# BurntSushi/suffix

Hardware: AMD Instinct MI355X
Metric: MB of input text/sec for SuffixTable::new (SA-IS+LCP), 1 GPU; bit-exact SA (higher is better)
Workload: dtype u32; 1 GPU; 100000000 B synthetic DNA (sigma=4, uniform, splitmix64) per GPU, u32 indices, device-resident text -> device SA; text_bytes_total=100000000

## Files before the change

### suffix_amd/csrc/sfx_host.hpp

```cpp
#pragma once
#include <cstring>
#include <hip/hip_runtime.h>
#include <stdint.h>
#include <stdlib.h>

#include "../../include/suffix_hip.h"
#include "sfx_device.hpp"

namespace sfx {

void note_hip_error(hipError_t e, const char* what, const char* file, int line);

#define SFX_HIP(expr)                                                   \
    do {                                                                \
        hipError_t e_ = (expr);                                         \
        if (e_ != hipSuccess) {                                         \
            ::sfx::note_hip_error(e_, #expr, __FILE__, __LINE__);       \
            return SFX_ERR_HIP;                                         \
        }                                                               \
    } while (0)

#define SFX_TRY(expr)                       \
    do {                                    \
        int s_ = (expr);                    \
// ... 43 lines not shown
};
inline unsigned grid_cap()
{
    static const unsigned cap = [] {
        const char* e = dev_env("SFX_MAX_GRID");
        int v = e ? atoi(e) : 0;
        return (v >= 1 && v <= (int)kMaxGrid) ? (unsigned)v : kMaxGrid;
    }();
    return cap;
}
inline Chunking make_chunking(uint64_t items, uint64_t tile, unsigned max_blocks = kMaxGrid)
{
    Chunking c;
    if (max_blocks > grid_cap()) max_blocks = grid_cap();
    c.tiles = (items + tile - 1) / tile;
    if (c.tiles == 0) c.tiles = 1;
    c.tiles_per_block = (c.tiles + max_blocks - 1) / max_blocks;
    c.blocks = (unsigned)((c.tiles + c.tiles_per_block - 1) / c.tiles_per_block);
    return c;
}

bool profile_on();
void profile_begin(const char* name, hipStream_t st, double algo_bytes);
void profile_end(hipStream_t st);

#define SFX_LAUNCH(name, algo_bytes, kernel, grid, block, stream, ...)                  \
    do {                                                                                \
        if (::sfx::profile_on()) ::sfx::profile_begin(name, stream, (double)(algo_bytes)); \
        hipLaunchKernelGGL(kernel, dim3(grid), dim3(block), 0, stream, __VA_ARGS__);    \
        if (::sfx::profile_on()) ::sfx::profile_end(stream);                            \
        SFX_HIP(hipGetLastError());                                                     \
    } while (0)

#ifndef SFX_EMULATED
namespace detail {
constexpr unsigned kPostWords = 64;
static __global__ void __launch_bounds__(64) k_post_words(const uint32_t* __restrict__ src, unsigned words, volatile uint32_t* host,
                                                   uint32_t seq)
{
    const unsigned lane = threadIdx.x;
    if (lane < words) host[lane] = src[lane];
    __threadfence_system();
    __builtin_amdgcn_s_waitcnt(0);
    if (lane == 0) host[kPostWords] = seq;
}
}
#endif
inline int read_back(void* dst, const void* d_src, size_t bytes, hipStream_t st)
{
    constexpr size_t kStage = 4096, kPostArea = 512;
    thread_local void* stage = nullptr;
    thread_local bool tried = false;
    if (!tried) {
        tried = true;
        if (hipHostMalloc(&stage, kStage + kPostArea, hipHostMallocPortable | hipHostMallocMapped | hipHostMallocCoherent) != hipSuccess) {
            stage = nullptr;
            (void)hipGetLastError();
        }
        if (stage) std::memset(stage, 0, kStage + kPostArea);
    }
#ifndef SFX_EMULATED
    thread_local uint32_t seq = 0;
    if (stage && bytes > 0 && bytes <= detail::kPostWords * 4 && (bytes & 3u) == 0 && (reinterpret_cast<uintptr_t>(d_src) & 3u) == 0) {
        static_assert((detail::kPostWords + 16) * 4 <= kPostArea, "payload + the sequence word's own 64-byte block");
        volatile uint32_t* const host = reinterpret_cast<volatile uint32_t*>(static_cast<char*>(stage) + kStage);
        if (++seq == 0) seq = 1;
        hipLaunchKernelGGL(detail::k_post_words, dim3(1), dim3(64), 0, st, static_cast<const uint32_t*>(d_src), (unsigned)(bytes / 4), host, seq);
        SFX_HIP(hipGetLastError());
        for (unsigned spins = 1;; spins++) {
            if (host[detail::kPostWords] == seq) break;
#if defined(__x86_64__) || defined(__i386__)
            __builtin_ia32_pause();
#endif
            if ((spins & 0xFFFu) == 0) {
                const hipError_t q = hipStreamQuery(st);
                if (q == hipErrorNotReady) continue;
                SFX_HIP(q);
                if (host[detail::kPostWords] == seq) break;
                SFX_HIP(hipStreamSynchronize(st));
                goto by_copy;
            }
        }
        for (size_t i = 0; i < bytes / 4; i++) static_cast<uint32_t*>(dst)[i] = host[i];
        return SFX_OK;
    }
by_copy:
#endif
    void* via = (stage && bytes <= kStage) ? stage : dst;
    SFX_HIP(hipMemcpyAsync(via, d_src, bytes, hipMemcpyDeviceToHost, st));
    SFX_HIP(hipStreamSynchronize(st));
    if (via != dst) std::memcpy(dst, via, bytes);
    return SFX_OK;
}

struct BuildStats;

uint64_t radix_scratch_words(uint64_t m);
struct TieRecords {
    bool produced;
    const uint32_t* tmask;
    uint32_t* lmask;
    uint32_t* hmask;
    bool want_keys;
};
int radix_sort_e64(uint64_t* e0, uint64_t* e1, uint64_t m, int bit_lo, int bit_hi, uint32_t* scratch,
                   hipStream_t st, int* result_in_1, sfx_build_stats* stats, const PackedText* text,
                   uint32_t* split_v, uint32_t** split_k_out, unsigned hist_blocks = 0, int elem_bits = 0, TieRecords* ties = nullptr);
unsigned radix_e64_presort_hist(uint64_t m, int bit_lo, int bit_hi);
bool radix_e64_hybrid_expected(uint64_t m, int key_bits);
inline uint32_t* radix_partial(uint32_t* scratch) { return scratch; }
int radix_sort_kv64(uint64_t* k0, uint32_t* v0, uint64_t* k1, uint32_t* v1, uint64_t m, int bit_lo,
                    int bit_hi, uint32_t* scratch, hipStream_t st, int* result_in_1,
                    sfx_build_stats* stats, const PackedText* text, uint32_t* last_v = nullptr, uint64_t kv12_cap = 0);
int radix_sort_ht64(uint64_t* k0, uint32_t* v0, uint64_t* k1, uint32_t* v1, uint64_t m, uint32_t* scratch, hipStream_t st,
                    int* result_in_1, sfx_build_stats* stats, const PackedText& text, const uint32_t* ht, uint32_t* last_v = nullptr,
                    uint64_t kv12_cap = 0, int ctx_sigma = 0);
struct LcpEmit;
struct SegSort {
    void* segs;
    void* tiles;
    uint32_t* tilehist;
    uint32_t* segexcl;
    uint32_t* status;
    uint64_t status_words;
    uint32_t* counters;
// ... 165 lines not shown
```

### suffix_amd/csrc/sfx_radix.hip

```cpp
#include <stdio.h>
#include <type_traits>
#include <stdlib.h>

#include "sfx_host.hpp"

namespace sfx {

constexpr uint32_t kStatusAgg = 1u << 30;
constexpr uint32_t kStatusPrefix = 2u << 30;
constexpr uint32_t kStatusValue = (1u << 30) - 1u;
constexpr int kMaxPasses = 8;
constexpr unsigned kHistAllGrid = 1024;

struct SrcE64 {
    static constexpr bool kHasVal = false;
    static constexpr bool kFromText = false;
    const uint64_t* in;
    __device__ __forceinline__ uint64_t key(uint64_t i) const { return in[i]; }
    __device__ __forceinline__ uint32_t val(uint64_t) const { return 0u; }
};
struct SrcText32 {
    static constexpr bool kHasVal = false;
    static constexpr bool kFromText = true;
    PackedText t;
    __device__ __forceinline__ uint64_t key(uint64_t i) const
    {
        return ((uint64_t)packed_key32(t, i) << 32) | (uint64_t)(uint32_t)i;
    }
    __device__ __forceinline__ uint32_t val(uint64_t) const { return 0u; }
};
struct SrcText36 {
    static constexpr bool kHasVal = false;
    static constexpr bool kFromText = true;
    PackedText t;
    int extra;
    bool wide;
    __device__ __forceinline__ uint64_t key(uint64_t i) const
    {
        uint64_t k64;
        if (wide) {
            k64 = packed_key64(t, i);
        } else {
            const uint64_t q = packed_word_index(t, i);
            const unsigned off = packed_word_offset(t, i, q);
            uint64_t pair;
            __builtin_memcpy(&pair, t.words + q, 8);
            const uint64_t both = ((pair & 0xFFFFFFFFull) << 32) | (pair >> 32);
            k64 = both << (off * (unsigned)t.bits);
        }
        return ((k64 >> (32 - extra)) << (32 - extra)) | (uint64_t)(uint32_t)i;
    }
    __device__ __forceinline__ uint32_t val(uint64_t) const { return 0u; }
};
struct SrcKV {
    static constexpr bool kHasVal = true;
    static constexpr bool kFromText = false;
    const uint64_t* k;
    const uint32_t* v;
    __device__ __forceinline__ uint64_t key(uint64_t i) const { return k[i]; }
    __device__ __forceinline__ uint32_t val(uint64_t i) const { return v[i]; }
};
struct SrcKeyIota {
    static constexpr bool kHasVal = true;
    static constexpr bool kFromText = false;
    const uint64_t* k;
    __device__ __forceinline__ uint64_t key(uint64_t i) const { return k[i]; }
    __device__ __forceinline__ uint32_t val(uint64_t i) const { return (uint32_t)i; }
};
struct SrcText64 {
    static constexpr bool kHasVal = true;
    static constexpr bool kFromText = true;
    PackedText t;
    __device__ __forceinline__ uint64_t key(uint64_t i) const { return packed_key64(t, i); }
    __device__ __forceinline__ uint32_t val(uint64_t i) const { return (uint32_t)i; }
};
struct DstE64 {
    uint64_t* out;
    __device__ __forceinline__ void store(uint32_t d, uint64_t key, uint32_t) const { out[d] = key; }
};
struct DstSplit32 {
    uint32_t* k;
    uint32_t* v;
    __device__ __forceinline__ void store(uint32_t d, uint64_t key, uint32_t) const
    {
        k[d] = (uint32_t)(key >> 32);
// ... 680 lines not shown
#pragma unroll
                for (int j = 0; j < kOut; j++) {
                    ok[j] = s.stage[(j0 + j) * kThreads + t];
                    ov[j] = HAS_VAL ? s.stage_v[(j0 + j) * kThreads + t] : 0u;
                }
#pragma unroll
                for (int j = 0; j < kOut; j++) od[j] = s.off[digit_of(ok[j], shift, mask)] + (unsigned)(h * kHalf + (j0 + j) * kThreads) + t;
#pragma unroll
                for (int j = 0; j < kOut; j++)
                    if ((unsigned)(h * kHalf + (j0 + j) * kThreads) + t < nvalid) dst.store(od[j], ok[j], ov[j]);
            }
        }
        if (owner) {
            unsigned col = tid;
            SFX_OPAQUE_VGPR(col);
#pragma unroll
            for (int k = 0; k < NW; k++) s.cnt[k][col] = 0;
        }
        __syncthreads();
    }
}

constexpr unsigned kCursorPad = 16;
constexpr unsigned kPartClasses = 8;
template <int KPT, int NW>
struct PartSmem {
    uint64_t stage[NW * kWave * KPT];
    uint16_t cnt[NW][kRadix];
    uint32_t off[kRadix];
    uint32_t tiles_before[kRadix];
    uint32_t class_tiles[8];
    uint32_t part[2][NW];
};
template <class Src, int KPT, int NW, bool SUB>
__global__ void __launch_bounds__(NW * kWave) SFX_WAVES_PER_EU(4, 4)
k_partition(Src src, uint64_t* __restrict__ out, uint64_t m, int shift, uint32_t* __restrict__ cursor,
            const uint32_t* __restrict__ bstart16, uint64_t class_len)
{
    constexpr int kThreads = NW * kWave;
    constexpr uint32_t kTile = kThreads * KPT;
    static_assert(kThreads >= kRadix, "thread d owns bucket d");
    static_assert(kWave * KPT >= kRadix, "the match masks must fit the staging buffer");
    static_assert(kTile < 65536, "16-bit tile positions");
    __shared__ PartSmem<KPT, NW> s;
    const unsigned tid = threadIdx.x, lane = lane_id(), w = wave_id();
    const unsigned long long mybit = 1ull << lane;
    const bool owner = tid < (unsigned)kRadix;
    unsigned par = 0;
    unsigned long long* const my_flags = reinterpret_cast<unsigned long long*>(s.stage) + w * kRadix;
    uint64_t ntiles;
    {
        const uint64_t first = dmin<uint64_t>(m, class_len);
        ntiles = ((first + kTile - 1) / kTile) * kPartClasses;
    }
    if (SUB) {
        if (owner) s.tiles_before[tid] = (bstart16[(tid + 1u) << 8] - bstart16[tid << 8] + kTile - 1u) / kTile;
        __syncthreads();
        if (tid < 8u) {
            uint32_t run = 0;
            for (unsigned b = tid; b < (unsigned)kRadix; b += 8u) {
                const uint32_t tb = s.tiles_before[b];
                s.tiles_before[b] = run;
                run += tb;
            }
            s.class_tiles[tid] = run;
        }
        __syncthreads();
        uint32_t most = 0;
#pragma unroll
        for (int x = 0; x < 8; x++) most = dmax(most, s.class_tiles[x]);
        ntiles = (uint64_t)most * 8u;
    }
    if (owner) {
#pragma unroll
        for (int k = 0; k < NW; k++) s.cnt[k][tid] = 0;
    }
    __syncthreads();
    auto locate = [&](uint64_t v, uint64_t& begin, unsigned& nvalid, unsigned& top) {
        begin = v * kTile;
        nvalid = 0;
        top = 0;
        if (v >= ntiles) return;
        if (SUB) {
            const unsigned x = (unsigned)(v & 7u);
            const uint32_t u = (uint32_t)(v >> 3);
            if (u >= s.class_tiles[x]) return;
            unsigned lo = 0, hi = kRadix / 8;
            while (hi - lo > 1u) {
                const unsigned mid = (lo + hi) / 2u;
                if (s.tiles_before[x + 8u * mid] <= u) lo = mid; else hi = mid;
            }
            top = x + 8u * lo;
            const uint32_t b0 = bstart16[top << 8], b1 = bstart16[(top + 1u) << 8];
            begin = (uint64_t)b0 + (uint64_t)(u - s.tiles_before[top]) * kTile;
            nvalid = (unsigned)dmin<uint64_t>(kTile, (uint64_t)b1 - begin);
        } else {
            const unsigned x = (unsigned)(v % kPartClasses);
            const uint64_t p0 = dmin<uint64_t>(m, (uint64_t)x * class_len), p1 = dmin<uint64_t>(m, p0 + class_len);
            begin = p0 + (v / kPartClasses) * kTile;
            top = x;
            if (begin < p1) nvalid = (unsigned)dmin<uint64_t>(kTile, p1 - begin);
        }
    };
    for (uint64_t v = blockIdx.x; v < ntiles; v += gridDim.x) {
        uint64_t begin;
        unsigned nvalid, top;
        locate(v, begin, nvalid, top);
        if (nvalid == 0u) continue;
        uint64_t key[KPT];
        uint32_t pos[KPT];
        unsigned first = w * (kWave * KPT) + lane;
        SFX_OPAQUE_VGPR(first);
#pragma unroll
        for (int r = 0; r < KPT; r++) {
            const unsigned idx = first + r * kWave;
            key[r] = idx < nvalid ? src.key(begin + idx) : ~0ull;
        }
#pragma unroll
        for (int k = 0; k < kRadix / kWave; k++) my_flags[k * kWave + lane] = 0ull;
        wave_sync();
#pragma unroll
        for (int r = 0; r < KPT; r++) pos[r] = rank_round16(digit_of(key[r], shift, 255u), my_flags, s.cnt[w], mybit);
        __syncthreads();
        uint32_t real_count = 0, tile_ex = 0, mine = 0;
        {
            uint32_t c[NW], tile_count = 0;
#pragma unroll
            for (int k = 0; k < NW; k++) {
                c[k] = owner ? s.cnt[k][tid] : 0u;
                tile_count += c[k];
            }
            const uint32_t ex = block_scan_excl_1b<NW>(tile_count, s.part, par);
            if (owner) {
                uint32_t run = ex;
#pragma unroll
                for (int k = 0; k < NW; k++) {
                    s.cnt[k][tid] = (uint16_t)run;
                    run += c[k];
                }
                real_count = tile_count - ((tid == 255u) ? (uint32_t)(kTile - nvalid) : 0u);
                tile_ex = ex;
                if (real_count) mine = atomicAdd(&cursor[SUB ? ((top << 8) | tid) : (top * kRadix + tid) * kCursorPad], real_count);
            }
        }
        __syncthreads();
#pragma unroll
        for (int r = 0; r < KPT; r++) s.stage[pos[r] + s.cnt[w][digit_of(key[r], shift, 255u)]] = key[r];
        if (owner) s.off[tid] = mine - tile_ex;
        __syncthreads();
        constexpr int kOut = (KPT % 4 == 0) ? 4 : ((KPT % 2 == 0) ? 2 : 1);
        unsigned t = tid;
        SFX_OPAQUE_VGPR(t);
#pragma unroll
        for (int r0 = 0; r0 < KPT; r0 += kOut) {
#pragma unroll
            for (int r = r0; r < r0 + kOut; r++) key[r] = s.stage[r * kThreads + t];
#pragma unroll
            for (int r = r0; r < r0 + kOut; r++) pos[r] = s.off[digit_of(key[r], shift, 255u)] + ((unsigned)r * kThreads + t);
#pragma unroll
            for (int r = r0; r < r0 + kOut; r++)
                if ((unsigned)r * kThreads + t < nvalid) out[pos[r]] = key[r];
        }
        if (owner) {
#pragma unroll
            for (int k = 0; k < NW; k++) s.cnt[k][tid] = 0;
        }
        __syncthreads();
    }
}
__global__ void __launch_bounds__(kBlock)
k_partition_cursors(const uint32_t* __restrict__ bstart16, const uint32_t* __restrict__ class_top8, uint32_t* __restrict__ cursor16,
                    uint32_t* __restrict__ cursor8)
{
    const unsigned i = blockIdx.x * kBlock + threadIdx.x;
    if (i < (unsigned)(1 << 16)) {
        const uint32_t b = bstart16[i];
        cursor16[i] = b;
        if ((i & 255u) == 0u) {
            uint32_t run = b;
            for (unsigned x = 0; x < kPartClasses; x++) {
                cursor8[(x * kRadix + (i >> 8)) * kCursorPad] = run;
                run += class_top8[x * kRadix + (i >> 8)];
            }
        }
    }
}

constexpr int kH16Bins = 1 << 16;
constexpr int kH16Words = kH16Bins / 2;
constexpr int kH16Threads = 1024;
__global__ void __launch_bounds__(kH16Threads)
k_hist16_text(PackedText t, int drop, uint64_t words_per_block, uint32_t* __restrict__ partial)
{
    __shared__ uint32_t h[kH16Words];
    const unsigned tid = threadIdx.x;
    const uint64_t nwords = (t.n + (uint64_t)t.spw - 1) / (uint64_t)t.spw;
    const uint64_t qb = (uint64_t)blockIdx.x * words_per_block;
    const uint64_t qe = dmin<uint64_t>(nwords, qb + words_per_block);
    const uint64_t mask = (1ull << t.kbits) - 1ull;
    for (unsigned i = tid; i < (unsigned)kH16Words; i += kH16Threads) h[i] = 0;
    __syncthreads();
    for (uint64_t q = qb + tid; q < qe; q += kH16Threads) {
        const uint64_t both = ((uint64_t)t.words[q] << t.kbits) | (uint64_t)t.words[q + 1];
        const uint64_t j0 = q * (uint64_t)t.spw;
        for (int o = 0; o < t.spw; o++) {
            if (j0 + (uint64_t)o >= t.n) break;
            const uint32_t key = (uint32_t)((both >> ((unsigned)(t.spw - o) * (unsigned)t.bits)) & mask);
            const uint32_t top = key >> drop;
            atomicAdd(&h[top >> 1], (top & 1u) ? 65536u : 1u);
        }
    }
    __syncthreads();
    uint32_t* out = partial + (uint64_t)blockIdx.x * kH16Words;
    for (unsigned i = tid; i < (unsigned)kH16Words; i += kH16Threads) out[i] = h[i];
}
__global__ void __launch_bounds__(kH16Threads)
k_hist16_e64(const uint64_t* __restrict__ E, uint64_t m, int shift, uint64_t per_block, uint32_t* __restrict__ partial)
{
    __shared__ uint32_t h[kH16Words];
    const unsigned tid = threadIdx.x;
    const uint64_t qb = (uint64_t)blockIdx.x * per_block;
    const uint64_t qe = dmin<uint64_t>(m, qb + per_block);
    for (unsigned i = tid; i < (unsigned)kH16Words; i += kH16Threads) h[i] = 0;
    __syncthreads();
    constexpr int kFly = 8;
    for (uint64_t q0 = qb; q0 < qe; q0 += (uint64_t)kH16Threads * kFly) {
        uint64_t e[kFly];
#pragma unroll
        for (int k = 0; k < kFly; k++) {
            const uint64_t q = q0 + (uint64_t)k * kH16Threads + tid;
            e[k] = q < qe ? E[q] : ~0ull;
        }
#pragma unroll
        for (int k = 0; k < kFly; k++) {
            if (q0 + (uint64_t)k * kH16Threads + tid < qe) {
                const uint32_t top = (uint32_t)(e[k] >> shift) & 0xFFFFu;
                atomicAdd(&h[top >> 1], (top & 1u) ? 65536u : 1u);
            }
        }
    }
    __syncthreads();
    uint32_t* out = partial + (uint64_t)blockIdx.x * kH16Words;
    for (unsigned i = tid; i < (unsigned)kH16Words; i += kH16Threads) out[i] = h[i];
}
constexpr int kH16ReduceBins = 1024;
constexpr unsigned kH16ReduceSplit = 8;
__global__ void __launch_bounds__(kBlock)
k_hist16_reduce(const uint32_t* __restrict__ partial, unsigned nblocks, uint32_t* __restrict__ bins, unsigned rows_per_class,
                uint32_t* __restrict__ class_top8)
{
    const unsigned bx = blockIdx.x % (kH16Bins / kH16ReduceBins), by = blockIdx.x / (kH16Bins / kH16ReduceBins);
    const unsigned w0 = bx * (kH16ReduceBins / 2) + threadIdx.x * 2;
    uint32_t c[4] = {0, 0, 0, 0};
    const unsigned g1 = dmin(nblocks, (by + 1u) * rows_per_class);
    for (unsigned g = by * rows_per_class; g < g1; g++) {
        const uint2 v = *reinterpret_cast<const uint2*>(partial + (uint64_t)g * kH16Words + w0);
        c[0] += v.x & 0xFFFFu;
        c[1] += v.x >> 16;
        c[2] += v.y & 0xFFFFu;
        c[3] += v.y >> 16;
    }
#pragma unroll
    for (int k = 0; k < 4; k++)
        if (c[k]) atomicAdd(&bins[2 * w0 + k], c[k]);
    uint32_t all = c[0] + c[1] + c[2] + c[3];
    for (int d = 32; d >= 1; d >>= 1) all += __shfl_xor(all, d);
    static_assert(kWave * 4 == kRadix, "a wave's bins are one top-8 bucket");
    if (lane_id() == 0) class_top8[by * kRadix + (2u * w0) / (unsigned)kRadix] = all;
}
struct OversizeEntry { uint32_t bin, start, size, off; };
constexpr uint32_t kOversizeMax = 16384;
__global__ void __launch_bounds__(kH16Threads)
k_hist16_scan(uint32_t* __restrict__ bins, uint32_t* __restrict__ totals_lo, uint32_t* __restrict__ totals_hi,
              uint32_t* __restrict__ stat_out, uint32_t cap, uint32_t fast)
{
    __shared__ uint32_t part[kH16Threads / kWave];
    __shared__ uint32_t pmax[kH16Threads / kWave];
    __shared__ uint32_t lo[4][kRadix];
    __shared__ uint32_t tsum[kH16Threads];
    constexpr int kPer = kH16Bins / kH16Threads;
    const unsigned tid = threadIdx.x;
    {
        const unsigned d = tid & 255u, q = tid >> 8;
        uint32_t t = 0;
        for (unsigned j = q; j < (unsigned)kRadix; j += 4) t += bins[j * kRadix + d];
        lo[q][d] = t;
    }
    uint32_t v[kPer], sum = 0, most = 0;
    {
        uint32_t slow = 0, nover = 0, sover = 0;
        for (int j = 0; j < kPer; j++) {
            v[j] = bins[tid * kPer + j];
            sum += v[j];
            most = dmax(most, v[j]);
            if (v[j] > fast) slow += v[j];
            if (v[j] > cap) { nover++; sover += v[j]; }
        }
        if (slow) atomicAdd(&stat_out[4], slow);
        if (nover) { atomicAdd(&stat_out[2], nover); atomicAdd(&stat_out[3], sover); }
    }
    tsum[tid] = sum;
    for (int d = 32; d >= 1; d >>= 1) most = dmax(most, __shfl_xor(most, d));
    const uint32_t incl = wave_scan_add(sum);
    if (lane_id() == 63) part[wave_id()] = incl;
    if (lane_id() == 0) pmax[wave_id()] = most;
    __syncthreads();
    if (tid < (unsigned)kRadix) {
        totals_lo[tid] = lo[0][tid] + lo[1][tid] + lo[2][tid] + lo[3][tid];
        totals_hi[tid] = tsum[4 * tid] + tsum[4 * tid + 1] + tsum[4 * tid + 2] + tsum[4 * tid + 3];
    }
    uint32_t base = 0;
    for (unsigned k = 0; k < wave_id(); k++) base += part[k];
    uint32_t run = base + incl - sum;
    for (int j = 0; j < kPer; j++) { bins[tid * kPer + j] = run; run += v[j]; }
    if (tid == kH16Threads - 1) { bins[kH16Bins] = run; stat_out[1] = run; }
    if (tid == 0) {
        uint32_t mx = 0;
        for (unsigned k = 0; k < (unsigned)(kH16Threads / kWave); k++) mx = dmax(mx, pmax[k]);
        stat_out[0] = mx;
    }
}
__global__ void __launch_bounds__(kH16Threads)
k_hist16_oversize(const uint32_t* __restrict__ bstart, uint32_t cap, OversizeEntry* __restrict__ over)
{
    __shared__ uint64_t pover[kH16Threads / kWave];
    constexpr int kPer = kH16Bins / kH16Threads;
    const unsigned tid = threadIdx.x;
    uint64_t ov = 0;
    for (int j = 0; j < kPer; j++) {
        const uint32_t b = tid * kPer + j, v = bstart[b + 1] - bstart[b];
        if (v > cap) ov += (1ull << 32) | (uint64_t)v;
    }
    const uint64_t incl = wave_scan_add(ov);
    if (lane_id() == 63) pover[wave_id()] = incl;
    __syncthreads();
    uint64_t run = incl - ov;
    for (unsigned k = 0; k < wave_id(); k++) run += pover[k];
    if (ov == 0) return;
    for (int j = 0; j < kPer; j++) {
        const uint32_t b = tid * kPer + j, start = bstart[b], v = bstart[b + 1] - start;
        if (v > cap) {
            const uint32_t at = (uint32_t)(run >> 32);
            if (at < kOversizeMax) over[at] = OversizeEntry{b, start, v, (uint32_t)run};
            run += (1ull << 32) | (uint64_t)v;
        }
    }
}
__global__ void __launch_bounds__(kBlock)
k_oversize_gather(const uint64_t* __restrict__ X, const OversizeEntry* __restrict__ over, uint32_t nover, int low_bits,
                  uint64_t* __restrict__ T)
{
    const uint32_t lmask = (uint32_t)((1ull << low_bits) - 1ull);
// ... 374 lines not shown
bool radix_e64_hybrid_expected(uint64_t m, int key_bits)
{
    return hybrid_size_ok(m) && key_bits >= 24;
}
static int hybrid_sort_e64_text(uint64_t* e0, uint64_t* e1, uint64_t m, int bit_lo, int bit_hi, const RadixScratch& scr,
                                hipStream_t st, sfx_build_stats* stats, const PackedText& text, uint32_t* split_v,
                                uint32_t** split_k_out, bool* done, bool* windows_ready, int elem_bits = 0, TieRecords* ties = nullptr)
{
    if (ties) ties->produced = false;
    *done = false;
    *windows_ready = false;
    const bool from_elems = elem_bits > 0;
    static const uint32_t cap = [] {
        const char* e = dev_env("SFX_HYBRID_CAP");
        const uint32_t full = kBucketNW * kWave * kBucketKPT;
        const uint32_t v = e ? (uint32_t)atoi(e) : full;
        return v >= 1 && v < full ? v : full;
    }();
    const int key_bits = from_elems ? elem_bits : bit_hi - bit_lo;
    if (!hybrid_size_ok(m) || bit_lo != 32 || key_bits < 24 || key_bits > bit_hi - bit_lo) return SFX_OK;
    if (!from_elems && (key_bits != text.kbits || m != text.n)) return SFX_OK;
    const int low_bits = key_bits - 16;
    const int top_hi = bit_lo + key_bits;
    constexpr uint64_t kReserve = 1u << 18;
    uint32_t* bins = scr.partial + ((uint64_t)kMaxPasses * kRadix * kHistAllGrid - kReserve);
    uint32_t* stat = bins + kH16Bins + 64;
    OversizeEntry* over = reinterpret_cast<OversizeEntry*>(bins + kH16Bins + 128);
    static_assert(kH16Bins + 128 + 4 * kOversizeMax <= kReserve, "the reserve holds bins, statistics and the oversize list");
    uint32_t* partial = reinterpret_cast<uint32_t*>(e1);
    const uint64_t nwords = from_elems ? m : (m + (uint64_t)text.spw - 1) / (uint64_t)text.spw;
    const uint64_t room = m * sizeof(uint64_t) / (kH16Words * sizeof(uint32_t));
    if (room == 0) return SFX_OK;
    Chunking ch = make_chunking(nwords, kH16Threads, (unsigned)dmin<uint64_t>(room, 256));
    SFX_HIP(hipMemsetAsync(scr.tickets, 0, 64 * sizeof(uint32_t), st));
    SFX_HIP(hipMemsetAsync(bins, 0, (kH16Bins + 128) * sizeof(uint32_t), st));
    if (from_elems)
        SFX_LAUNCH("radix_hist16_elems", (double)m * 8.0, k_hist16_e64, ch.blocks, kH16Threads, st, (const uint64_t*)e0, m, top_hi - 16,
                   ch.tiles_per_block * kH16Threads, partial);
    else
        SFX_LAUNCH("radix_hist16_text", (double)m * text.bits / 8.0, k_hist16_text, ch.blocks, kH16Threads, st, text, low_bits,
                   ch.tiles_per_block * kH16Threads, partial);
    static_assert(kH16ReduceSplit == kPartClasses, "one block group of the reduction per stretch");
    const unsigned rows_per_class = (ch.blocks + kPartClasses - 1) / kPartClasses;
    const uint64_t class_len = (uint64_t)rows_per_class * ch.tiles_per_block * kH16Threads * (from_elems ? 1u : (uint64_t)text.spw);
    uint32_t* cursor16 = bins + kH16Bins + 128 + 4 * kOversizeMax;
    uint32_t* class_top8 = cursor16 + kH16Bins;
    uint32_t* cursor8 = class_top8 + kPartClasses * kRadix;
    static_assert(kH16Bins + 128 + 4 * kOversizeMax + kH16Bins + kPartClasses * kRadix * (1 + kCursorPad) <= kReserve, "the reserve holds the cursors too");
    SFX_LAUNCH("radix_hist16_reduce", (double)ch.blocks * kH16Words * 4, k_hist16_reduce, (kH16Bins / kH16ReduceBins) * kH16ReduceSplit, kBlock, st,
               (const uint32_t*)partial, ch.blocks, bins, rows_per_class, class_top8);
    SFX_LAUNCH("radix_hist16_scan", (double)kH16Bins * 8, k_hist16_scan, 1, kH16Threads, st, bins, scr.totals, scr.totals + kRadix,
               stat, cap, dmin(cap, 4096u));
    uint32_t host_stat[5] = {0, 0, 0, 0, 0};
    SFX_TRY(read_back(host_stat, stat, sizeof(host_stat), st));
    const uint32_t host_max = host_stat[0], nover = host_stat[2];
    const uint64_t nlarge = host_stat[3], nslow = host_stat[4];
    const bool give_way = nover > kOversizeMax || nslow * 64 > m ||
                          (nover && (m + 1) / 2 + 32 + 2 * (nlarge + 32) > m);
    if ((uint64_t)host_stat[1] != m) return SFX_OK;
    if (give_way) {
        if (!from_elems && text.kbits == 32 && (8 % text.bits) == 0 && bit_hi == 64) {
            SFX_HIP(hipMemsetAsync(scr.tickets, 0, 64 * sizeof(uint32_t), st));
            SFX_LAUNCH("radix_window_from_hist16", 0.0, k_window_from_hist16, 1, kBlock, st, scr.totals, (uint32_t)(3 * (8 / text.bits)));
            SFX_LAUNCH("radix_window_fix", 0.0, k_window_fix, 1, kBlock, st, text, scr.totals);
            *windows_ready = true;
        }
        return SFX_OK;
    }
    static const int ties_on = [] { const char* e = dev_env("SFX_HYBRID_TIES"); return e ? atoi(e) : 1; }();
    const bool tie_mode = ties && ties_on && nover == 0;
    static const int partition = [] { const char* e = dev_env("SFX_HYBRID_PARTITION"); return e ? atoi(e) : 1; }();
    static const int key36_on = [] { const char* e = dev_env("SFX_HYBRID_KEY36"); return e ? atoi(e) : 1; }();
    int extra = 0;
    if (tie_mode && key36_on && partition && !from_elems && text.kbits == 32 && text.bits <= 4 && m <= (1ull << 28))
        extra = key36_on >= 2 ? (4 / text.bits) * text.bits : text.bits;
    const bool wide_key = extra > text.bits;
    const int sbits = 32 - extra;
    if (partition) {
        constexpr int kPKpt = 16;
        SFX_LAUNCH("partition_cursors", (double)kH16Bins * 8, k_partition_cursors, kH16Bins / kBlock, kBlock, st, (const uint32_t*)bins,
                   (const uint32_t*)class_top8, cursor16, cursor8);
        static const unsigned cus = [] {
            int dev = 0, n = 0;
            if (hipGetDevice(&dev) != hipSuccess || hipDeviceGetAttribute(&n, hipDeviceAttributeMultiprocessorCount, dev) != hipSuccess || n <= 0) n = 256;
            return (unsigned)n;
        }();
        static const int pwaves = [] { const char* e = dev_env("SFX_PARTITION_WAVES"); const int v = e ? atoi(e) : 8; return (v == 16 || v == 4) ? v : 8; }();
        auto partition_pair = [&](auto nw) -> int {
            constexpr int kPNw = decltype(nw)::value;
            const uint64_t tile = (uint64_t)kPKpt * kPNw * kWave;
            const unsigned per_cu = 16u / kPNw;
            const unsigned g1 = (unsigned)dmin<uint64_t>((m + tile - 1) / tile, dmin(per_cu * cus, grid_cap()));
            const unsigned g2 = (unsigned)dmin<uint64_t>((m + tile - 1) / tile + kRadix, dmin(per_cu * cus, grid_cap()));
            if (from_elems) {
                SFX_LAUNCH("radix_scatter_u32", (double)m * 16.0, (k_partition<SrcE64, kPKpt, kPNw, false>), g1, kPNw * kWave, st,
                           SrcE64{e0}, e1, m, top_hi - 8, cursor8, (const uint32_t*)bins, class_len);
                SFX_LAUNCH("radix_scatter_u32", (double)m * 16.0, (k_partition<SrcE64, kPKpt, kPNw, true>), g2, kPNw * kWave, st,
                           SrcE64{e1}, e0, m, top_hi - 16, cursor16, (const uint32_t*)bins, class_len);
                uint64_t* t = e0; e0 = e1; e1 = t;
            } else {
                if (extra)
                    SFX_LAUNCH("radix_scatter_text_u32", (double)m * (text.bits / 8.0 + 8.0), (k_partition<SrcText36, kPKpt, kPNw, false>),
                               g1, kPNw * kWave, st, SrcText36{text, extra, wide_key}, e0, m, top_hi - 8, cursor8, (const uint32_t*)bins, class_len);
                else
                    SFX_LAUNCH("radix_scatter_text_u32", (double)m * (text.bits / 8.0 + 8.0), (k_partition<SrcText32, kPKpt, kPNw, false>),
                               g1, kPNw * kWave, st, SrcText32{text}, e0, m, top_hi - 8, cursor8, (const uint32_t*)bins, class_len);
                SFX_LAUNCH("radix_scatter_u32", (double)m * 16.0, (k_partition<SrcE64, kPKpt, kPNw, true>), g2, kPNw * kWave, st,
                           SrcE64{e0}, e1, m, top_hi - 16, cursor16, (const uint32_t*)bins, class_len);
            }
            return SFX_OK;
        };
        if (pwaves == 16) SFX_TRY(partition_pair(std::integral_constant<int, 16>{}));
        else if (pwaves == 4) SFX_TRY(partition_pair(std::integral_constant<int, 4>{}));
        else SFX_TRY(partition_pair(std::integral_constant<int, 8>{}));
    } else if (from_elems) {
        SFX_TRY(run_pass("radix_scatter_u32", (double)m * 16.0, SrcE64{e0}, DstE64{e1}, m, top_hi - 16, 255u, scr, 0, true, st));
        SFX_TRY(run_pass("radix_scatter_u32", (double)m * 16.0, SrcE64{e1}, DstE64{e0}, m, top_hi - 8, 255u, scr, 1, true, st));
        uint64_t* t = e0; e0 = e1; e1 = t;
    } else {
        SrcText32 tsrc = {text};
        SFX_TRY(run_pass("radix_scatter_text_u32", (double)m * (text.bits / 8.0 + 8.0), tsrc, DstE64{e0}, m, top_hi - 16, 255u, scr, 0,
                         true, st));
        SFX_TRY(run_pass("radix_scatter_u32", (double)m * 16.0, SrcE64{e0}, DstE64{e1}, m, top_hi - 8, 255u, scr, 1, true, st));
    }
    uint32_t* split_k = reinterpret_cast<uint32_t*>(e0);
    const uint64_t* over_sorted = nullptr;
    if (nover) {
        SFX_LAUNCH("radix_hist16_oversize", (double)kH16Bins * 8, k_hist16_oversize, 1, kH16Threads, st, (const uint32_t*)bins, cap, over);
        uint64_t* T = e0 + (((m + 1) / 2 + 31) & ~uint64_t(31));
        uint64_t* T2 = T + ((nlarge + 31) & ~uint64_t(31));
        const unsigned g = (unsigned)dmin<uint64_t>(nover, kMaxGrid);
        SFX_LAUNCH("oversize_gather", (double)nlarge * 16, k_oversize_gather, g, kBlock, st, (const uint64_t*)e1, (const OversizeEntry*)over,
                   nover, low_bits, T);
        int in1 = 0;
        SFX_TRY(radix_sort_e64(T, T2, nlarge, 32, 32 + low_bits + bits_for(nover > 1 ? nover - 1 : 1), scr.partial, st, &in1, stats,
                               nullptr, nullptr, nullptr, 0));
        over_sorted = in1 ? T2 : T;
    }
    static const int force_geom = [] { const char* e = dev_env("SFX_HYBRID_GEOM"); return e ? atoi(e) : -1; }();
// ... 681 lines not shown
```

Baseline: 76350 MB/s.

## Fuse radix hist16 reduce, scan and cursor setup; prefetch text words in partition

```diff
diff --git a/suffix_amd/csrc/sfx_host.hpp b/suffix_amd/csrc/sfx_host.hpp
--- a/suffix_amd/csrc/sfx_host.hpp
+++ b/suffix_amd/csrc/sfx_host.hpp
@@ -99,9 +99,11 @@
         SFX_HIP(hipGetLastError());                                                     \
     } while (0)
 
+namespace detail {
+constexpr unsigned kPostWords = 64;
+}
 #ifndef SFX_EMULATED
 namespace detail {
-constexpr unsigned kPostWords = 64;
 static __global__ void __launch_bounds__(64) k_post_words(const uint32_t* __restrict__ src, unsigned words, volatile uint32_t* host,
                                                    uint32_t seq)
 {
@@ -113,9 +115,14 @@
 }
 }
 #endif
-inline int read_back(void* dst, const void* d_src, size_t bytes, hipStream_t st)
-{
-    constexpr size_t kStage = 4096, kPostArea = 512;
+struct PostTicket {
+    volatile uint32_t* host;
+    uint32_t seq;
+};
+namespace detail {
+constexpr size_t kStage = 4096, kPostArea = 512;
+inline void* post_stage()
+{
     thread_local void* stage = nullptr;
     thread_local bool tried = false;
     if (!tried) {
@@ -126,14 +133,48 @@
         }
         if (stage) std::memset(stage, 0, kStage + kPostArea);
     }
+    return stage;
+}
+}
+inline PostTicket post_ticket()
+{
 #ifndef SFX_EMULATED
     thread_local uint32_t seq = 0;
-    if (stage && bytes > 0 && bytes <= detail::kPostWords * 4 && (bytes & 3u) == 0 && (reinterpret_cast<uintptr_t>(d_src) & 3u) == 0) {
-        static_assert((detail::kPostWords + 16) * 4 <= kPostArea, "payload + the sequence word's own 64-byte block");
-        volatile uint32_t* const host = reinterpret_cast<volatile uint32_t*>(static_cast<char*>(stage) + kStage);
+    void* const stage = detail::post_stage();
+    if (stage) {
+        static_assert((detail::kPostWords + 16) * 4 <= detail::kPostArea, "payload + the sequence word's own 64-byte block");
         if (++seq == 0) seq = 1;
-        hipLaunchKernelGGL(detail::k_post_words, dim3(1), dim3(64), 0, st, static_cast<const uint32_t*>(d_src), (unsigned)(bytes / 4), host, seq);
-        SFX_HIP(hipGetLastError());
+        return PostTicket{reinterpret_cast<volatile uint32_t*>(static_cast<char*>(stage) + detail::kStage), seq};
+    }
+#endif
+    return PostTicket{nullptr, 0};
+}
+template <class Words>
+__device__ __forceinline__ void post_words_from_kernel(const PostTicket& t, const Words& src, unsigned words)
+{
+#ifndef SFX_EMULATED
+    if (!t.host) return;
+    for (unsigned i = 0; i < words; i++) t.host[i] = src[i];
+    __threadfence_system();
+    __builtin_amdgcn_s_waitcnt(0);
+    t.host[detail::kPostWords] = t.seq;
+#endif
+}
+inline int read_by_copy(void* dst, const void* d_src, size_t bytes, hipStream_t st)
+{
+    void* const stage = detail::post_stage();
+    void* via = (stage && bytes <= detail::kStage) ? stage : dst;
+    SFX_HIP(hipMemcpyAsync(via, d_src, bytes, hipMemcpyDeviceToHost, st));
+    SFX_HIP(hipStreamSynchronize(st));
+    if (via != dst) std::memcpy(dst, via, bytes);
+    return SFX_OK;
+}
+inline int read_posted(void* dst, const void* d_src, size_t bytes, const PostTicket& t, hipStream_t st)
+{
+#ifndef SFX_EMULATED
+    if (t.host && bytes > 0 && bytes <= detail::kPostWords * 4 && (bytes & 3u) == 0) {
+        volatile uint32_t* const host = t.host;
+        const uint32_t seq = t.seq;
         for (unsigned spins = 1;; spins++) {
             if (host[detail::kPostWords] == seq) break;
 #if defined(__x86_64__) || defined(__i386__)
@@ -145,19 +186,29 @@
                 SFX_HIP(q);
                 if (host[detail::kPostWords] == seq) break;
                 SFX_HIP(hipStreamSynchronize(st));
-                goto by_copy;
+                return read_by_copy(dst, d_src, bytes, st);
             }
         }
         for (size_t i = 0; i < bytes / 4; i++) static_cast<uint32_t*>(dst)[i] = host[i];
         return SFX_OK;
     }
-by_copy:
-#endif
-    void* via = (stage && bytes <= kStage) ? stage : dst;
-    SFX_HIP(hipMemcpyAsync(via, d_src, bytes, hipMemcpyDeviceToHost, st));
-    SFX_HIP(hipStreamSynchronize(st));
-    if (via != dst) std::memcpy(dst, via, bytes);
-    return SFX_OK;
+#endif
+    return read_by_copy(dst, d_src, bytes, st);
+}
+inline int read_back(void* dst, const void* d_src, size_t bytes, hipStream_t st)
+{
+#ifndef SFX_EMULATED
+    if (bytes > 0 && bytes <= detail::kPostWords * 4 && (bytes & 3u) == 0 && (reinterpret_cast<uintptr_t>(d_src) & 3u) == 0) {
+        const PostTicket t = post_ticket();
+        if (t.host) {
+            hipLaunchKernelGGL(detail::k_post_words, dim3(1), dim3(64), 0, st, static_cast<const uint32_t*>(d_src), (unsigned)(bytes / 4), t.host,
+                               t.seq);
+            SFX_HIP(hipGetLastError());
+            return read_posted(dst, d_src, bytes, t, st);
+        }
+    }
+#endif
+    return read_by_copy(dst, d_src, bytes, st);
 }
 
 struct BuildStats;
diff --git a/suffix_amd/csrc/sfx_radix.hip b/suffix_amd/csrc/sfx_radix.hip
--- a/suffix_amd/csrc/sfx_radix.hip
+++ b/suffix_amd/csrc/sfx_radix.hip
@@ -28,6 +28,10 @@
         return ((uint64_t)packed_key32(t, i) << 32) | (uint64_t)(uint32_t)i;
     }
     __device__ __forceinline__ uint32_t val(uint64_t) const { return 0u; }
+    __device__ __forceinline__ uint64_t from_window(uint64_t k64, uint64_t i) const
+    {
+        return (k64 & 0xFFFFFFFF00000000ull) | (uint64_t)(uint32_t)i;
+    }
 };
 struct SrcText36 {
     static constexpr bool kHasVal = false;
@@ -48,9 +52,37 @@
             const uint64_t both = ((pair & 0xFFFFFFFFull) << 32) | (pair >> 32);
             k64 = both << (off * (unsigned)t.bits);
         }
+        return from_window(k64, i);
+    }
+    __device__ __forceinline__ uint32_t val(uint64_t) const { return 0u; }
+    __device__ __forceinline__ uint64_t from_window(uint64_t k64, uint64_t i) const
+    {
         return ((k64 >> (32 - extra)) << (32 - extra)) | (uint64_t)(uint32_t)i;
     }
-    __device__ __forceinline__ uint32_t val(uint64_t) const { return 0u; }
+};
+template <int SPW, int KPT>
+struct TextTileWords {
+    static_assert(SPW >= KPT ? SPW % KPT == 0 : KPT % SPW == 0, "a thread's positions begin on a word boundary or stay inside one word");
+    static constexpr int kOwn = SPW >= KPT ? 1 : KPT / SPW;
+    static constexpr int kCount = kOwn + 1;
+    uint32_t w[kCount];
+    __device__ __forceinline__ void load(const PackedText& t, uint64_t begin, unsigned tid)
+    {
+        __builtin_memcpy(w, t.words + (begin / (unsigned)SPW + ((uint64_t)tid * KPT) / (unsigned)SPW), sizeof(w));
+    }
+    template <class Src>
+    __device__ __forceinline__ void keys(const Src& src, uint64_t begin, unsigned tid, uint64_t (&key)[KPT]) const
+    {
+        constexpr unsigned kBits = 32u / SPW;
+        const unsigned off0 = SPW > KPT ? (tid * KPT) % (unsigned)SPW : 0u;
+#pragma unroll
+        for (int r = 0; r < KPT; r++) {
+            const int j = SPW > KPT ? 0 : r / SPW;
+            const unsigned off = SPW > KPT ? off0 + (unsigned)r : (unsigned)(r % SPW);
+            const uint64_t both = ((uint64_t)w[j] << 32) | (uint64_t)w[j + 1];
+            key[r] = src.from_window(both << (off * kBits), begin + (uint64_t)tid * KPT + (unsigned)r);
+        }
+    }
 };
 struct SrcKV {
     static constexpr bool kHasVal = true;
@@ -797,13 +829,14 @@
     uint32_t class_tiles[8];
     uint32_t part[2][NW];
 };
-template <class Src, int KPT, int NW, bool SUB>
+template <class Src, int KPT, int NW, bool SUB, int SPW = 0>
 __global__ void __launch_bounds__(NW * kWave) SFX_WAVES_PER_EU(4, 4)
 k_partition(Src src, uint64_t* __restrict__ out, uint64_t m, int shift, uint32_t* __restrict__ cursor,
             const uint32_t* __restrict__ bstart16, uint64_t class_len)
 {
     constexpr int kThreads = NW * kWave;
     constexpr uint32_t kTile = kThreads * KPT;
+    static_assert(SPW == 0 || (Src::kFromText && !SUB), "the tile loader reads packed text");
     static_assert(kThreads >= kRadix, "thread d owns bucket d");
     static_assert(kWave * KPT >= kRadix, "the match masks must fit the staging buffer");
     static_assert(kTile < 65536, "16-bit tile positions");
@@ -867,19 +900,42 @@
             if (begin < p1) nvalid = (unsigned)dmin<uint64_t>(kTile, p1 - begin);
         }
     };
+    TextTileWords<SPW ? SPW : KPT, KPT> words = {};
+    auto request = [&](uint64_t v) {
+        if constexpr (SPW > 0) {
+            uint64_t begin;
+            unsigned nvalid, top;
+            locate(v, begin, nvalid, top);
+            if (nvalid == kTile) words.load(src.t, begin, tid);
+        }
+    };
+    request(blockIdx.x);
     for (uint64_t v = blockIdx.x; v < ntiles; v += gridDim.x) {
         uint64_t begin;
         unsigned nvalid, top;
         locate(v, begin, nvalid, top);
-        if (nvalid == 0u) continue;
+        if (nvalid == 0u) {
+            request(v + gridDim.x);
+            continue;
+        }
         uint64_t key[KPT];
         uint32_t pos[KPT];
-        unsigned first = w * (kWave * KPT) + lane;
-        SFX_OPAQUE_VGPR(first);
-#pragma unroll
-        for (int r = 0; r < KPT; r++) {
-            const unsigned idx = first + r * kWave;
-            key[r] = idx < nvalid ? src.key(begin + idx) : ~0ull;
+        bool striped = true;
+        if constexpr (SPW > 0) {
+            if (nvalid == kTile) {
+                words.keys(src, begin, tid, key);
+                striped = false;
+            }
+            request(v + gridDim.x);
+        }
+        if (striped) {
+            unsigned first = w * (kWave * KPT) + lane;
+            SFX_OPAQUE_VGPR(first);
+#pragma unroll
+            for (int r = 0; r < KPT; r++) {
+                const unsigned idx = first + r * kWave;
+                key[r] = idx < nvalid ? src.key(begin + idx) : ~0ull;
+            }
         }
 #pragma unroll
         for (int k = 0; k < kRadix / kWave; k++) my_flags[k * kWave + lane] = 0ull;
@@ -933,30 +989,24 @@
         __syncthreads();
     }
 }
-__global__ void __launch_bounds__(kBlock)
-k_partition_cursors(const uint32_t* __restrict__ bstart16, const uint32_t* __restrict__ class_top8, uint32_t* __restrict__ cursor16,
-                    uint32_t* __restrict__ cursor8)
-{
-    const unsigned i = blockIdx.x * kBlock + threadIdx.x;
-    if (i < (unsigned)(1 << 16)) {
-        const uint32_t b = bstart16[i];
-        cursor16[i] = b;
-        if ((i & 255u) == 0u) {
-            uint32_t run = b;
-            for (unsigned x = 0; x < kPartClasses; x++) {
-                cursor8[(x * kRadix + (i >> 8)) * kCursorPad] = run;
-                run += class_top8[x * kRadix + (i >> 8)];
-            }
-        }
-    }
-}
-
 constexpr int kH16Bins = 1 << 16;
 constexpr int kH16Words = kH16Bins / 2;
 constexpr int kH16Threads = 1024;
+struct H16Zero {
+    uint32_t* a;
+    uint32_t na;
+    uint32_t* b;
+    uint32_t nb;
+    __device__ __forceinline__ void clear(unsigned threads) const
+    {
+        for (uint32_t i = blockIdx.x * threads + threadIdx.x; i < na; i += gridDim.x * threads) a[i] = 0;
+        for (uint32_t i = blockIdx.x * threads + threadIdx.x; i < nb; i += gridDim.x * threads) b[i] = 0;
+    }
+};
 __global__ void __launch_bounds__(kH16Threads)
-k_hist16_text(PackedText t, int drop, uint64_t words_per_block, uint32_t* __restrict__ partial)
-{
+k_hist16_text(PackedText t, int drop, uint64_t words_per_block, uint32_t* __restrict__ partial, H16Zero z)
+{
+    z.clear(kH16Threads);
     __shared__ uint32_t h[kH16Words];
     const unsigned tid = threadIdx.x;
     const uint64_t nwords = (t.n + (uint64_t)t.spw - 1) / (uint64_t)t.spw;
@@ -965,8 +1015,11 @@
     const uint64_t mask = (1ull << t.kbits) - 1ull;
     for (unsigned i = tid; i < (unsigned)kH16Words; i += kH16Threads) h[i] = 0;
     __syncthreads();
+    uint32_t w0 = 0, w1 = 0;
+    if (qb + tid < qe) { w0 = t.words[qb + tid]; w1 = t.words[qb + tid + 1]; }
     for (uint64_t q = qb + tid; q < qe; q += kH16Threads) {
-        const uint64_t both = ((uint64_t)t.words[q] << t.kbits) | (uint64_t)t.words[q + 1];
+        const uint64_t both = ((uint64_t)w0 << t.kbits) | (uint64_t)w1;
+        if (q + kH16Threads < qe) { w0 = t.words[q + kH16Threads]; w1 = t.words[q + kH16Threads + 1]; }
         const uint64_t j0 = q * (uint64_t)t.spw;
         for (int o = 0; o < t.spw; o++) {
             if (j0 + (uint64_t)o >= t.n) break;
@@ -980,8 +1033,9 @@
     for (unsigned i = tid; i < (unsigned)kH16Words; i += kH16Threads) out[i] = h[i];
 }
 __global__ void __launch_bounds__(kH16Threads)
-k_hist16_e64(const uint64_t* __restrict__ E, uint64_t m, int shift, uint64_t per_block, uint32_t* __restrict__ partial)
-{
+k_hist16_e64(const uint64_t* __restrict__ E, uint64_t m, int shift, uint64_t per_block, uint32_t* __restrict__ partial, H16Zero z)
+{
+    z.clear(kH16Threads);
     __shared__ uint32_t h[kH16Words];
     const unsigned tid = threadIdx.x;
     const uint64_t qb = (uint64_t)blockIdx.x * per_block;
@@ -1008,81 +1062,132 @@
     uint32_t* out = partial + (uint64_t)blockIdx.x * kH16Words;
     for (unsigned i = tid; i < (unsigned)kH16Words; i += kH16Threads) out[i] = h[i];
 }
-constexpr int kH16ReduceBins = 1024;
-constexpr unsigned kH16ReduceSplit = 8;
-__global__ void __launch_bounds__(kBlock)
-k_hist16_reduce(const uint32_t* __restrict__ partial, unsigned nblocks, uint32_t* __restrict__ bins, unsigned rows_per_class,
-                uint32_t* __restrict__ class_top8)
-{
-    const unsigned bx = blockIdx.x % (kH16Bins / kH16ReduceBins), by = blockIdx.x / (kH16Bins / kH16ReduceBins);
-    const unsigned w0 = bx * (kH16ReduceBins / 2) + threadIdx.x * 2;
-    uint32_t c[4] = {0, 0, 0, 0};
-    const unsigned g1 = dmin(nblocks, (by + 1u) * rows_per_class);
-    for (unsigned g = by * rows_per_class; g < g1; g++) {
-        const uint2 v = *reinterpret_cast<const uint2*>(partial + (uint64_t)g * kH16Words + w0);
-        c[0] += v.x & 0xFFFFu;
-        c[1] += v.x >> 16;
-        c[2] += v.y & 0xFFFFu;
-        c[3] += v.y >> 16;
-    }
-#pragma unroll
-    for (int k = 0; k < 4; k++)
-        if (c[k]) atomicAdd(&bins[2 * w0 + k], c[k]);
-    uint32_t all = c[0] + c[1] + c[2] + c[3];
-    for (int d = 32; d >= 1; d >>= 1) all += __shfl_xor(all, d);
-    static_assert(kWave * 4 == kRadix, "a wave's bins are one top-8 bucket");
-    if (lane_id() == 0) class_top8[by * kRadix + (2u * w0) / (unsigned)kRadix] = all;
-}
 struct OversizeEntry { uint32_t bin, start, size, off; };
 constexpr uint32_t kOversizeMax = 16384;
-__global__ void __launch_bounds__(kH16Threads)
-k_hist16_scan(uint32_t* __restrict__ bins, uint32_t* __restrict__ totals_lo, uint32_t* __restrict__ totals_hi,
-              uint32_t* __restrict__ stat_out, uint32_t cap, uint32_t fast)
-{
-    __shared__ uint32_t part[kH16Threads / kWave];
-    __shared__ uint32_t pmax[kH16Threads / kWave];
-    __shared__ uint32_t lo[4][kRadix];
-    __shared__ uint32_t tsum[kH16Threads];
-    constexpr int kPer = kH16Bins / kH16Threads;
+constexpr int kH16FinThreads = 512;
+constexpr int kH16FinBins = 4 * kH16FinThreads;
+constexpr int kH16FinHalf = kH16Bins / 2;
+constexpr int kH16FinPer = kH16FinHalf / kH16FinThreads;
+__global__ void __launch_bounds__(kH16FinThreads)
+k_hist16_finish(const uint32_t* __restrict__ partial, unsigned nblocks, unsigned rows_per_class, uint32_t* bins,
+                uint32_t* class_top8, uint32_t* ticket, uint32_t* __restrict__ totals_lo, uint32_t* __restrict__ totals_hi,
+                uint32_t* __restrict__ stat_out, uint32_t cap, uint32_t fast, uint32_t* __restrict__ cursor16,
+                uint32_t* __restrict__ cursor8, PostTicket post)
+{
+    constexpr int kWaves = kH16FinThreads / kWave;
+    __shared__ uint32_t tile[kH16FinHalf + kH16FinHalf / kH16FinPer];
+    __shared__ uint32_t lo[kRadix];
+    __shared__ uint32_t part[kWaves];
+    __shared__ uint32_t sstat[5];
+    __shared__ uint32_t last;
     const unsigned tid = threadIdx.x;
     {
-        const unsigned d = tid & 255u, q = tid >> 8;
-        uint32_t t = 0;
-        for (unsigned j = q; j < (unsigned)kRadix; j += 4) t += bins[j * kRadix + d];
-        lo[q][d] = t;
-    }
-    uint32_t v[kPer], sum = 0, most = 0;
-    {
-        uint32_t slow = 0, nover = 0, sover = 0;
-        for (int j = 0; j < kPer; j++) {
-            v[j] = bins[tid * kPer + j];
-            sum += v[j];
-            most = dmax(most, v[j]);
-            if (v[j] > fast) slow += v[j];
-            if (v[j] > cap) { nover++; sover += v[j]; }
-        }
-        if (slow) atomicAdd(&stat_out[4], slow);
-        if (nover) { atomicAdd(&stat_out[2], nover); atomicAdd(&stat_out[3], sover); }
-    }
-    tsum[tid] = sum;
-    for (int d = 32; d >= 1; d >>= 1) most = dmax(most, __shfl_xor(most, d));
-    const uint32_t incl = wave_scan_add(sum);
-    if (lane_id() == 63) part[wave_id()] = incl;
-    if (lane_id() == 0) pmax[wave_id()] = most;
+        constexpr unsigned kGroups = kH16Bins / kH16FinBins;
+        const unsigned bx = blockIdx.x % kGroups, by = blockIdx.x / kGroups;
+        const unsigned w0 = bx * (kH16FinBins / 2) + tid * 2;
+        uint32_t c[4] = {0, 0, 0, 0};
+        const unsigned g1 = dmin(nblocks, (by + 1u) * rows_per_class);
+        constexpr int kFly = 4;
+        for (unsigned g = by * rows_per_class; g < g1; g += kFly) {
+            uint2 v[kFly];
+#pragma unroll
+            for (int k = 0; k < kFly; k++) {
+                v[k] = uint2{0u, 0u};
+                if (g + (unsigned)k < g1) v[k] = *reinterpret_cast<const uint2*>(partial + (uint64_t)(g + (unsigned)k) * kH16Words + w0);
+            }
+#pragma unroll
+            for (int k = 0; k < kFly; k++) {
+                c[0] += v[k].x & 0xFFFFu;
+                c[1] += v[k].x >> 16;
+                c[2] += v[k].y & 0xFFFFu;
+                c[3] += v[k].y >> 16;
+            }
+        }
+#pragma unroll
+        for (int k = 0; k < 4; k++)
+            if (c[k]) atomicAdd(&bins[2 * w0 + k], c[k]);
+        uint32_t all = c[0] + c[1] + c[2] + c[3];
+        for (int d = 32; d >= 1; d >>= 1) all += __shfl_xor(all, d);
+        static_assert(kWave * 4 == kRadix, "a wave's bins are one top-8 bucket");
+        if (lane_id() == 0) class_top8[by * kRadix + (2u * w0) / (unsigned)kRadix] = all;
+    }
+    __builtin_amdgcn_fence(__ATOMIC_RELEASE, "agent");
     __syncthreads();
-    if (tid < (unsigned)kRadix) {
-        totals_lo[tid] = lo[0][tid] + lo[1][tid] + lo[2][tid] + lo[3][tid];
-        totals_hi[tid] = tsum[4 * tid] + tsum[4 * tid + 1] + tsum[4 * tid + 2] + tsum[4 * tid + 3];
-    }
-    uint32_t base = 0;
-    for (unsigned k = 0; k < wave_id(); k++) base += part[k];
-    uint32_t run = base + incl - sum;
-    for (int j = 0; j < kPer; j++) { bins[tid * kPer + j] = run; run += v[j]; }
-    if (tid == kH16Threads - 1) { bins[kH16Bins] = run; stat_out[1] = run; }
+    if (tid == 0) last = (atomicAdd(ticket, 1u) == gridDim.x - 1u) ? 1u : 0u;
+    __syncthreads();
+    if (!last) return;
+    __builtin_amdgcn_fence(__ATOMIC_ACQUIRE, "agent");
+    if (tid < (unsigned)kRadix) lo[tid] = 0;
+    if (tid < 5u) sstat[tid] = 0;
+    uint32_t lo4[4] = {0, 0, 0, 0}, carry = 0;
+    uint32_t most = 0, slow = 0, nover = 0, sover = 0;
+    auto padded = [](unsigned i) { return i + i / (unsigned)kH16FinPer; };
+    for (int h = 0; h < 2; h++) {
+        uint32_t* const src = bins + h * kH16FinHalf;
+        __syncthreads();
+#pragma unroll 4
+        for (int k = 0; k < kH16FinPer / 4; k++) {
+            const unsigned i = (unsigned)k * kH16FinBins + 4u * tid;
+            const uint4 v = *reinterpret_cast<const uint4*>(src + i);
+            lo4[0] += v.x; lo4[1] += v.y; lo4[2] += v.z; lo4[3] += v.w;
+            const unsigned at = padded(i);
+            tile[at] = v.x; tile[at + 1] = v.y; tile[at + 2] = v.z; tile[at + 3] = v.w;
+        }
+        __syncthreads();
+        uint32_t* const mine = tile + padded(tid * kH16FinPer);
+        uint32_t sum = 0;
+        for (int j = 0; j < kH16FinPer; j++) {
+            const uint32_t x = mine[j];
+            sum += x;
+            most = dmax(most, x);
+            if (x > fast) slow += x;
+            if (x > cap) { nover++; sover += x; }
+        }
+        const uint32_t incl = wave_scan_add(sum);
+        if (lane_id() == 63) part[wave_id()] = incl;
+        __syncthreads();
+        uint32_t run = carry + incl - sum, total = 0;
+        for (unsigned k = 0; k < (unsigned)kWaves; k++) {
+            if (k < wave_id()) run += part[k];
+            total += part[k];
+        }
+        carry += total;
+        static_assert(kRadix % kH16FinPer == 0, "a top-8 bucket begins with a thread's first bin");
+        if ((tid * kH16FinPer) % (unsigned)kRadix == 0u) {
+            const unsigned j = ((unsigned)h * kH16FinHalf + tid * kH16FinPer) / (unsigned)kRadix;
+            uint32_t at = run;
+            for (unsigned x = 0; x < kPartClasses; x++) {
+                cursor8[(x * kRadix + j) * kCursorPad] = at;
+                at += class_top8[x * kRadix + j];
+            }
+            totals_hi[j] = at - run;
+        }
+        for (int j = 0; j < kH16FinPer; j++) {
+            const uint32_t x = mine[j];
+            mine[j] = run;
+            run += x;
+        }
+        __syncthreads();
+#pragma unroll 4
+        for (int k = 0; k < kH16FinPer / 4; k++) {
+            const unsigned i = (unsigned)k * kH16FinBins + 4u * tid, at = padded(i);
+            const uint4 v = uint4{tile[at], tile[at + 1], tile[at + 2], tile[at + 3]};
+            *reinterpret_cast<uint4*>(src + i) = v;
+            *reinterpret_cast<uint4*>(cursor16 + h * kH16FinHalf + i) = v;
+        }
+    }
+#pragma unroll
+    for (int k = 0; k < 4; k++) atomicAdd(&lo[(4u * tid + (unsigned)k) % (unsigned)kRadix], lo4[k]);
+    atomicMax(&sstat[0], most);
+    if (slow) atomicAdd(&sstat[4], slow);
+    if (nover) { atomicAdd(&sstat[2], nover); atomicAdd(&sstat[3], sover); }
+    __syncthreads();
+    if (tid < (unsigned)kRadix) totals_lo[tid] = lo[tid];
     if (tid == 0) {
-        uint32_t mx = 0;
-        for (unsigned k = 0; k < (unsigned)(kH16Threads / kWave); k++) mx = dmax(mx, pmax[k]);
-        stat_out[0] = mx;
+        bins[kH16Bins] = carry;
+        const uint32_t words[5] = {sstat[0], carry, sstat[2], sstat[3], sstat[4]};
+        for (int k = 0; k < 5; k++) stat_out[k] = words[k];
+        post_words_from_kernel(post, words, 5u);
     }
 }
 __global__ void __launch_bounds__(kH16Threads)
@@ -1523,27 +1628,25 @@
     const uint64_t room = m * sizeof(uint64_t) / (kH16Words * sizeof(uint32_t));
     if (room == 0) return SFX_OK;
     Chunking ch = make_chunking(nwords, kH16Threads, (unsigned)dmin<uint64_t>(room, 256));
-    SFX_HIP(hipMemsetAsync(scr.tickets, 0, 64 * sizeof(uint32_t), st));
-    SFX_HIP(hipMemsetAsync(bins, 0, (kH16Bins + 128) * sizeof(uint32_t), st));
+    const H16Zero zero = {bins, (uint32_t)(kH16Bins + 128), scr.tickets, 64u};
     if (from_elems)
         SFX_LAUNCH("radix_hist16_elems", (double)m * 8.0, k_hist16_e64, ch.blocks, kH16Threads, st, (const uint64_t*)e0, m, top_hi - 16,
-                   ch.tiles_per_block * kH16Threads, partial);
+                   ch.tiles_per_block * kH16Threads, partial, zero);
     else
         SFX_LAUNCH("radix_hist16_text", (double)m * text.bits / 8.0, k_hist16_text, ch.blocks, kH16Threads, st, text, low_bits,
-                   ch.tiles_per_block * kH16Threads, partial);
-    static_assert(kH16ReduceSplit == kPartClasses, "one block group of the reduction per stretch");
+                   ch.tiles_per_block * kH16Threads, partial, zero);
     const unsigned rows_per_class = (ch.blocks + kPartClasses - 1) / kPartClasses;
     const uint64_t class_len = (uint64_t)rows_per_class * ch.tiles_per_block * kH16Threads * (from_elems ? 1u : (uint64_t)text.spw);
     uint32_t* cursor16 = bins + kH16Bins + 128 + 4 * kOversizeMax;
     uint32_t* class_top8 = cursor16 + kH16Bins;
     uint32_t* cursor8 = class_top8 + kPartClasses * kRadix;
     static_assert(kH16Bins + 128 + 4 * kOversizeMax + kH16Bins + kPartClasses * kRadix * (1 + kCursorPad) <= kReserve, "the reserve holds the cursors too");
-    SFX_LAUNCH("radix_hist16_reduce", (double)ch.blocks * kH16Words * 4, k_hist16_reduce, (kH16Bins / kH16ReduceBins) * kH16ReduceSplit, kBlock, st,
-               (const uint32_t*)partial, ch.blocks, bins, rows_per_class, class_top8);
-    SFX_LAUNCH("radix_hist16_scan", (double)kH16Bins * 8, k_hist16_scan, 1, kH16Threads, st, bins, scr.totals, scr.totals + kRadix,
-               stat, cap, dmin(cap, 4096u));
     uint32_t host_stat[5] = {0, 0, 0, 0, 0};
-    SFX_TRY(read_back(host_stat, stat, sizeof(host_stat), st));
+    const PostTicket post = post_ticket();
+    SFX_LAUNCH("radix_hist16_finish", (double)ch.blocks * kH16Words * 4 + (double)kH16Bins * 12, k_hist16_finish,
+               (kH16Bins / kH16FinBins) * kPartClasses, kH16FinThreads, st, (const uint32_t*)partial, ch.blocks, rows_per_class, bins, class_top8,
+               stat + 16, scr.totals, scr.totals + kRadix, stat, cap, dmin(cap, 4096u), cursor16, cursor8, post);
+    SFX_TRY(read_posted(host_stat, stat, sizeof(host_stat), post, st));
     const uint32_t host_max = host_stat[0], nover = host_stat[2];
     const uint64_t nlarge = host_stat[3], nslow = host_stat[4];
     const bool give_way = nover > kOversizeMax || nslow * 64 > m ||
@@ -1569,8 +1672,6 @@
     const int sbits = 32 - extra;
     if (partition) {
         constexpr int kPKpt = 16;
-        SFX_LAUNCH("partition_cursors", (double)kH16Bins * 8, k_partition_cursors, kH16Bins / kBlock, kBlock, st, (const uint32_t*)bins,
-                   (const uint32_t*)class_top8, cursor16, cursor8);
         static const unsigned cus = [] {
             int dev = 0, n = 0;
             if (hipGetDevice(&dev) != hipSuccess || hipDeviceGetAttribute(&n, hipDeviceAttributeMultiprocessorCount, dev) != hipSuccess || n <= 0) n = 256;
@@ -1590,12 +1691,25 @@
                            SrcE64{e1}, e0, m, top_hi - 16, cursor16, (const uint32_t*)bins, class_len);
                 uint64_t* t = e0; e0 = e1; e1 = t;
             } else {
-                if (extra)
-                    SFX_LAUNCH("radix_scatter_text_u32", (double)m * (text.bits / 8.0 + 8.0), (k_partition<SrcText36, kPKpt, kPNw, false>),
-                               g1, kPNw * kWave, st, SrcText36{text, extra, wide_key}, e0, m, top_hi - 8, cursor8, (const uint32_t*)bins, class_len);
-                else
-                    SFX_LAUNCH("radix_scatter_text_u32", (double)m * (text.bits / 8.0 + 8.0), (k_partition<SrcText32, kPKpt, kPNw, false>),
-                               g1, kPNw * kWave, st, SrcText32{text}, e0, m, top_hi - 8, cursor8, (const uint32_t*)bins, class_len);
+                const int loader_spw = (kPNw == 8 && text.bits * text.spw == 32 && text.kbits == 32 && !wide_key &&
+                                        class_len % (uint64_t)text.spw == 0) ? text.spw : 0;
+                auto text_pass = [&](auto tsrc, auto spw) -> int {
+                    SFX_LAUNCH("radix_scatter_text_u32", (double)m * (text.bits / 8.0 + 8.0),
+                               (k_partition<decltype(tsrc), kPKpt, kPNw, false, (kPNw == 8 ? decltype(spw)::value : 0)>), g1, kPNw * kWave, st,
+                               tsrc, e0, m, top_hi - 8, cursor8, (const uint32_t*)bins, class_len);
+                    return SFX_OK;
+                };
+                auto text_pass_of = [&](auto tsrc) -> int {
+                    switch (loader_spw) {
+                    case 32: return text_pass(tsrc, std::integral_constant<int, 32>{});
+                    case 16: return text_pass(tsrc, std::integral_constant<int, 16>{});
+                    case 8: return text_pass(tsrc, std::integral_constant<int, 8>{});
+                    case 4: return text_pass(tsrc, std::integral_constant<int, 4>{});
+                    default: return text_pass(tsrc, std::integral_constant<int, 0>{});
+                    }
+                };
+                if (extra) SFX_TRY(text_pass_of(SrcText36{text, extra, wide_key}));
+                else SFX_TRY(text_pass_of(SrcText32{text}));
                 SFX_LAUNCH("radix_scatter_u32", (double)m * 16.0, (k_partition<SrcE64, kPKpt, kPNw, true>), g2, kPNw * kWave, st,
                            SrcE64{e0}, e1, m, top_hi - 16, cursor16, (const uint32_t*)bins, class_len);
             }
```

Result: faster. 78350 MB/s, median of 6 (+2.6%).
